# Illumina/strelka

Measured on AMD Instinct MI355X. Metric: candidate-alignment scoring cells/s (read bases x candidate alignments; Strelka2 has no pair-HMM, SURVEY.md section 0) + germline loci/s + 40x WGS-like germline wall-clock (e2e) + 110x/40x somatic wall-clock (e2e_somatic), higher is better.
Workload: dtype f64; 1 GPU; germline chr20-style synthetic (BASELINE.json configs[1]).  Headline: scoreCandidateAlignment as one function -- per GPU per step 65536 reads of 150 bp x 87.9 candidate alignments each (5-7 candidate indels around them), from the candidate alignments the device search left (PCal) to one double each: one kernel (F5: the walk of each alignment's path + the terms of its bases, penalties and clips).  ; read_len=150

## Files before the change

strelka_amd/csrc/read_enumerate.hip:

```cpp

#include "sk_common.h"

#include "align_entry.h"
#include "read_enumerate.h"

#include <algorithm>
#include <chrono>
#include <climits>
#include <cstdio>
#include <cstdlib>
#include <cstring>
#include <vector>

using namespace skcore;

int sk_score_alignments_launch_hostleg(const sk_align_batch* b, double* dev_out_lnp, void* hip_stream);

namespace
{

static_assert(sizeof(PFrame) % 4 == 0 && sizeof(PCal) % 4 == 0, "frames move through LDS as 32-bit words");


struct EnumArgs
// ... 337 lines not shown
            if (k <= a.light_cals) a.list[lat++] = r; else a.list[n - 1 - hat++] = r;
        }
        atomicMax(&a.dyn[DYN_MAX_CALS], max_cals);
        if (t == 0) {
            a.dyn[DYN_N_CALS] = total;
            a.dyn[DYN_N_LIGHT] = tot_light;
            a.dyn[DYN_N_HEAVY] = tot_heavy;
        }
    }
}


__device__ inline uint8_t code_of(const char c)
{
    switch (c) {
    case '=': return SK_BAM_REF;
    case 'A': return SK_BAM_A;
    case 'C': return SK_BAM_C;
    case 'G': return SK_BAM_G;
    case 'T': return SK_BAM_T;
    default: return SK_BAM_ANY;
    }
}

struct FlatArgs
{
    PJob job;
    const char* ins_pool;
    const char* ref;
    int32_t ref_offset, ref_len;
    int32_t n_reads, n_cals;
    const PCal* pool;
    const int32_t* list;
    int32_t* status;
    const int64_t* read_off;
    const uint8_t* read_code;
    const int32_t* cal_off;
    int32_t* win_begin;
    int32_t* win_end;
    int32_t* ins_lo;
    int32_t* ins_hi;
    uint8_t* n_seg8;
    int32_t* win_len;
    int32_t* hap_len;
    int32_t* n_ins;
    int16_t* ins_idx;
    int32_t* ins_off;
    int32_t* n_ops;
    const int64_t* hap_off;
    PCal* cals;
    uint8_t* hap_code;
    const int64_t* op_off;
// ... 291 lines not shown
            s_cal[k * REC_STRIDE + j] = v;
            dst[j] = v;
        }
    }
    __syncthreads();
    if (c >= a.n_cals) return;
    const int r = read_of_cal(a, c);
    const PCal& cal = *reinterpret_cast<const PCal*>(s_cal + lane * REC_STRIDE);
    if (a.status[r] != ST_OK) return;
    (void)flatten_cal<true>(a, r, cal, int32_t(a.read_off[r + 1] - a.read_off[r]), a.ops + a.op_off[c]);
    for (int i = 0; i < cal.n_indels; ++i) (void)job_cand(a.job, cal.indels[i]);
    if (cal.lead >= 0) (void)job_cand(a.job, cal.lead);
    if (cal.trail >= 0) (void)job_cand(a.job, cal.trail);
}

constexpr int F5_MAX_READ = 256;
constexpr int ONE_WAIT_MAX_READS = 16384;
constexpr int F5_MAX_POOL = 768;
#ifndef F5_SORT
#define F5_SORT 1
#endif
constexpr int F5_TAB = 32;

static_assert(F5_TAB <= 64, "the table copy is a lane an entry");

struct FusedScoreArgs
{
    FlatArgs f;
    const uint8_t* read_qual;
    const SkTables* tab;
    double* scores;
    unsigned* err;
    int32_t* n_unhandled;
    int32_t write_cals;
    unsigned long long* dbg;
    unsigned* queue;
};

constexpr int F5_SEGS = 16, F5_INDELS = 8;
constexpr int F5_SLOT = (F5_SEGS + 1) | 1;
__device__ __forceinline__ int f5_ent_word(const int k) { return k; }
constexpr int F5_ROW = 3;

struct F5Tab
{
    int32_t pos;
    uint32_t del, ins_len;
    uint32_t type_cand;
    int32_t ins_at;
};

template <int MAXR>
struct F5Lds
{
    uint8_t read[MAXR + 12];
    uint8_t hap[F5_MAX_POOL + 12];
    double row[(MAXR + 8) * F5_ROW];
    uint32_t slot[64 * F5_SLOT];
    F5Tab tab[F5_TAB];
};
static_assert(sizeof(F5Lds<152>) <= 10240, "sixteen waves of the short-read form to a CU");
static_assert(3 * 4 * sizeof(F5Lds<F5_MAX_READ>) <= 160 * 1024, "three four-wave blocks of the long-read form to a CU");
static_assert((152 + 12) % 4 == 0 && (F5_MAX_READ + 12) % 4 == 0 && (F5_MAX_POOL + 12) % 4 == 0, "the byte arrays' words stay aligned");
static_assert(INS_CAP <= 64, "a lane an insert");

struct F5Rec
{
    uint32_t w0, w1, w2;
    uint64_t types;
    uint64_t l0, l1, l2, l3;
    uint64_t ind;
    int ind_lo;
    __device__ __forceinline__ int32_t pos() const { return int32_t(w0); }
    __device__ __forceinline__ int lead() const { return int(int16_t(w1 & 0xffffu)); }
    __device__ __forceinline__ int trail() const { return int(int16_t(w1 >> 16)); }
    __device__ __forceinline__ int n_seg() const { return int((w2 >> 8) & 0xffu); }
    __device__ __forceinline__ int n_indels() const { return int((w2 >> 16) & 0xffu); }
    __device__ __forceinline__ int indel(const int k) const { return ind_lo + int(unsigned(ind >> (6 * k)) & 63u); }
};
static_assert(F5_TAB <= 64 && 6 * F5_INDELS <= 64, "an indel index in 6 bits, eight in one value");

template <typename LDS>
__device__ __forceinline__ int f5_walk_selects(LDS& S, const F5Rec c, const bool has, const int tab_lo, const int32_t win_begin, uint8_t* consulted,
                                               const int32_t L, const int32_t P, uint32_t* const myslot)
{
    constexpr uint64_t N1 = 0x1111111111111111ull;
    const uint64_t types = c.types, p_l0 = c.l0, p_l1 = c.l1, p_l2 = c.l2, p_l3 = c.l3;
    const int aps = has ? c.n_seg() : 0;
    auto eq4 = [=](const unsigned v) -> uint64_t {
        uint64_t x = types ^ (N1 * v);
        x |= x >> 1;
        x |= x >> 2;
        return ~x & N1;
    };
    auto seg_len = [=](const int i) -> unsigned {
        const uint64_t lo = (i & 4) ? p_l1 : p_l0, hi = (i & 4) ? p_l3 : p_l2;
        return unsigned(((i & 8) ? hi : lo) >> (16 * (i & 3))) & 0xffffu;
    };
    const uint64_t in_path = (aps >= 16) ? N1 : (((1ull << (4 * aps)) - 1ull) & N1);
    const uint64_t M4 = (eq4(SK_SEG_MATCH) | eq4(SK_SEG_SEQ_MATCH) | eq4(SK_SEG_SEQ_MISMATCH)) & in_path;
    const uint64_t I4 = eq4(SK_SEG_INSERT) & in_path, D4 = eq4(SK_SEG_DELETE) & in_path;
    const int ends_first = M4 ? (__builtin_ctzll(M4) >> 2) : aps, ends_second = M4 ? ((63 - __builtin_clzll(M4)) >> 2) : aps;
    const int ni = c.n_indels();
    int ni_wave = 0;
#pragma unroll
    for (int k = 1; k <= F5_INDELS; ++k) ni_wave = __any(ni >= k) ? k : ni_wave;
// ... 44 lines not shown
                else del_len += l;
            }
            read_step = ins_len;
            ref_step = del_len;
        }
        const unsigned asked = (del_len << 16) | ins_len;
        const bool askable = del_len < 0xffffu && ins_len < 0xffffu;
        int k_found = 0, n_found = 0;
        bool open = true;
#pragma unroll
        for (int k = 0; k < F5_INDELS; ++k) {
            if (k < ni_wave) {
                const bool m = open && k_pos[k] == ref_head_pos && k_pack[k] == asked;
                k_found = m ? k : k_found;
                n_found += m ? 1 : 0;
                open = open && (m || k_pos[k] <= ref_head_pos);
            }
        }
        int key = (n_found == 1) ? c.indel(k_found) : -2;
        key = (pi < ends_first) ? c.lead() : (pi > ends_second) ? c.trail() : key;
        const bool key_ok = key >= 0;
        const F5Tab te = S.tab[(key_ok ? key : tab_lo) - tab_lo];
        const bool indel_ok = live && is_indel_seg && key_ok;
        if (indel_ok && consulted) consulted[key] = 1;
        const bool pen = is_indel_seg && (te.type_cand >> 8) == 0u;
        const int32_t head = (pi < ends_first) ? int32_t(te.ins_len) - int32_t(ln) : 0;
        const bool ins_bases = is_indel_seg && ins_len > 0u;
        const bool ins_ok = ins_len <= 0xffffu && head >= 0 && uint32_t(head) + ins_len <= te.ins_len && te.ins_at >= 0;
        const bool bases = ins_bases || is_match;
        const int32_t src = ins_bases ? te.ins_at + head : ref_head_pos - win_begin;
        const unsigned len = ins_bases ? ins_len : ln;
        const bool known = is_indel_seg || is_match || is_clip || ty == SK_SEG_SKIP || ty == SK_SEG_HARD_CLIP;
        bool fail = !known || (is_indel_seg && (!key_ok || !askable)) || (ins_bases && !ins_ok);
        const bool entry = (bases || (is_clip && !is_indel_seg)) && len > 0u;
        if (entry) {
            fail = fail || pos + int32_t(len) > L || (bases && (src < 0 || int64_t(src) + int64_t(len) > int64_t(P)));
            const int hidx = bases ? int(src) - pos : 0;
            fail = fail || n_ent > F5_SEGS || npen > 4u || hidx < -256 || hidx > 3839;
            if (live && !fail) myslot[f5_ent_word(n_ent)] = unsigned(pos) | (npen << 9) | (bases ? 0u : 1u << 15) | (unsigned(hidx + 256) << 16);
        }
        if (live) {
            bad = fail;
            n_ent += entry ? 1 : 0;
            npen = entry ? (pen ? 1u : 0u) : npen + (pen ? 1u : 0u);
            pos += int32_t(read_step);
            ref_head_pos += int32_t(ref_step);
            pi += n_seg;
// ... 63 lines not shown
            const unsigned base = __umul24(unsigned(8 * F5_ROW), unsigned(p));
            double v[8];
#pragma unroll
            for (int u = 0; u < 8; ++u) {
                const unsigned at = base + unsigned(8 * F5_ROW * u) + ((sel[u >> 2] >> (8 * (u & 3))) & 0xffu);
                v[u] = *reinterpret_cast<const double*>(rows + at);
            }
#pragma unroll
            for (int u = 0; u < 8; ++u) lnp = __dadd_rn(lnp, v[u]);
            p += mm;
        }
        if (next_op()) break;
    }
    return lnp;
}

__device__ __forceinline__ void f5_wave_sync()
{
    __builtin_amdgcn_fence(__ATOMIC_RELEASE, "workgroup");
    __builtin_amdgcn_wave_barrier();
    __builtin_amdgcn_fence(__ATOMIC_ACQUIRE, "workgroup");
}

template <int MAXR, bool TIMING>
__device__ __forceinline__ void f5_read(const FusedScoreArgs& fa, const int r, F5Lds<MAXR>& S)
{
    auto now = [&]() -> unsigned long long { return TIMING ? (unsigned long long)clock64() : 0ull; };
    const FlatArgs& a = fa.f;
    const int lane = threadIdx.x & 63;
    const int c0 = a.cal_off[r], c1 = a.cal_off[r + 1];
    const int ncr = c1 - c0;
    if (ncr == 0 || a.status[r] != ST_OK) return;
    unsigned long long stamp[8];
    stamp[0] = now();
    const unsigned long long wall0 = TIMING ? (unsigned long long)wall_clock64() : 0ull;
    for (int i = 1; i < 8; ++i) stamp[i] = 0;
    const int64_t ro = a.read_off[r];
    const int32_t L = int32_t(a.read_off[r + 1] - ro);
    const int32_t P = a.hap_len[r];
    if (L > MAXR || P > F5_MAX_POOL) {
        if (lane == 0) atomicAdd(fa.n_unhandled, 1);
        return;
    }
    const int32_t win_begin = a.win_begin[r];
    const int n_ins = a.n_ins[r];
    int my_ins_idx = -1;
    int32_t my_ins_off = 0;
    {
        const int16_t* idx = a.ins_idx + size_t(r) * INS_CAP;
        const int32_t* off = a.ins_off + size_t(r) * INS_CAP;
        int32_t my_ins_len = 0;
        uint32_t my_ins_src = 0;
        if (lane < n_ins) {
            const int t_idx = idx[lane];
            my_ins_idx = t_idx;
            my_ins_off = off[lane];
            my_ins_len = int32_t(a.job.tab[t_idx].ins_len);
            my_ins_src = a.job.tab[t_idx].ins_off;
        }
        const int32_t win_len = a.win_len[r];
        for (int32_t i = lane; i < P + 8; i += 64) {
            uint8_t v = SK_BAM_ANY;
            if (i < win_len) {
                const int32_t p = win_begin + i;
                const bool outside = (p < a.ref_offset || p >= a.ref_offset + a.ref_len);
                if (outside && a.ref_outside) atomicAdd(a.ref_outside, 1);
                v = outside ? uint8_t(SK_BAM_ANY) : code_of(a.ref[p - a.ref_offset]);
            }
            S.hap[i] = v;
        }
        f5_wave_sync();
        for (int k = 0; k < n_ins; ++k) {
            const int32_t o = __builtin_amdgcn_readlane(my_ins_off, k), n = __builtin_amdgcn_readlane(my_ins_len, k);
            const uint32_t src = uint32_t(__builtin_amdgcn_readlane(int(my_ins_src), k));
            for (int32_t i = lane; i < n; i += 64)
                if (o + i < P) S.hap[o + i] = code_of(a.ins_pool[src + uint32_t(i)]);
        }
        const SkTables* __restrict__ T = fa.tab;
        for (int32_t i = lane; i < L + 12; i += 64) {
            unsigned q = 0;
            uint8_t code = SK_BAM_ANY;
            if (i < L) {
                code = a.read_code[ro + i];
                q = fa.read_qual[ro + i];
                if (q > 70u) {
                    atomicOr(fa.err, unsigned(SK_DEVERR_QSCORE));
                    q = 70u;
                }
            }
            S.read[i] = code & 15u;
            if (i < L + 8) {
                const unsigned c = code & 15u;
                const bool adds = i < L && c != 15u;
                const double agree = adds ? T->q2lncompe[q] : 0.0;
                S.row[F5_ROW * i] = agree;
                S.row[F5_ROW * i + 1] = 0.0;
                S.row[F5_ROW * i + 2] = !adds ? 0.0 : (c == 0u) ? agree : T->q2mis[q];
            }
        }
    }
    const double ln_quarter = fa.tab->ln_quarter, ln_noncand = fa.tab->ln_noncand;

    uint8_t* const order = S.hap + ((P + 8 + 3) & ~3);
    const bool sorted_order = (F5_SORT != 0) && ncr > 64 && ncr <= 256 && ((P + 8 + 3) & ~3) + ncr <= int(sizeof(S.hap));
    if (sorted_order) {
        int seg_of[4];
#pragma unroll
        for (int k = 0; k < 4; ++k) {
            const int j = lane + 64 * k;
            seg_of[k] = (j < ncr) ? int(a.n_seg8[c0 + j]) : -1;
            seg_of[k] = min(seg_of[k], F5_SEGS + 1);
        }
        unsigned present = 0;
#pragma unroll
        for (int k = 0; k < 4; ++k) present |= (seg_of[k] >= 0) ? (1u << seg_of[k]) : 0u;
#pragma unroll
        for (int d = 32; d >= 1; d >>= 1) present |= unsigned(__shfl_xor(int(present), d));
        present = unsigned(__builtin_amdgcn_readfirstlane(int(present)));
        int at = 0;
        while (present != 0u) {
            const int v = 31 - __builtin_clz(present);
            present &= ~(1u << v);
#pragma unroll
            for (int k = 0; k < 4; ++k) {
                const uint64_t m = __ballot(seg_of[k] == v);
                if (seg_of[k] == v) order[at + __popcll(m & ((1ull << lane) - 1ull))] = uint8_t(lane + 64 * k);
                at += __popcll(m);
            }
        }
    }

    for (int j0 = 0; j0 < ncr; j0 += 64) {
        const int nc = min(64, ncr - j0);
        f5_wave_sync();
        const unsigned long long ta = now();
        if (j0 == 0) stamp[1] = ta;
        const bool has = lane < nc;
        uint32_t* const myslot = S.slot + lane * F5_SLOT;
        bool fits = true;
        const int my_j = has ? (sorted_order ? int(order[j0 + lane]) : j0 + lane) : 0;
        F5Rec rec;
        rec.w0 = rec.w1 = rec.w2 = 0;
        rec.types = 0;
        rec.l0 = rec.l1 = rec.l2 = rec.l3 = 0;
        rec.ind = 0;
        rec.ind_lo = 0;
        uint64_t ind_raw0 = 0, ind_raw1 = 0;
        if (has) {
            const PCal* src = a.pool + a.list[c0 + my_j];
            const uint4* s4 = reinterpret_cast<const uint4*>(src);
            const uint4 q0 = s4[0], q1 = s4[1], q2 = s4[2], q3 = s4[3], q4 = s4[4];
            const uint32_t* si = reinterpret_cast<const uint32_t*>(src->indels);
            const uint32_t i0 = si[0], i1 = si[1], i2 = si[2], i3 = si[3];
            ind_raw0 = uint64_t(i0) | (uint64_t(i1) << 32);
            ind_raw1 = uint64_t(i2) | (uint64_t(i3) << 32);
            rec.w0 = q0.x;
            rec.w1 = q0.y;
            rec.w2 = q0.z;
            const unsigned nseg = (q0.z >> 8) & 0xffu, nind = (q0.z >> 16) & 0xffu;
            fits = (nseg <= unsigned(F5_SEGS) && nind <= unsigned(F5_INDELS));
            uint64_t types = 0;
            bool odd_type = false;
            auto pack4 = [&](const uint32_t a0, const uint32_t a1, const uint32_t a2, const uint32_t a3, const int first) -> uint64_t {
                types |= (uint64_t(a0 & 15u) | (uint64_t(a1 & 15u) << 4) | (uint64_t(a2 & 15u) << 8) | (uint64_t(a3 & 15u) << 12)) << (4 * first);
                odd_type = odd_type || (unsigned(first) < nseg && (a0 & 0xffffu) > 15u) || (unsigned(first + 1) < nseg && (a1 & 0xffffu) > 15u) ||
                           (unsigned(first + 2) < nseg && (a2 & 0xffffu) > 15u) || (unsigned(first + 3) < nseg && (a3 & 0xffffu) > 15u);
                return uint64_t(a0 >> 16) | (uint64_t(a1 >> 16) << 16) | (uint64_t(a2 >> 16) << 32) | (uint64_t(a3 >> 16) << 48);
            };
            rec.l0 = pack4(q0.w, q1.x, q1.y, q1.z, 0);
            rec.l1 = pack4(q1.w, q2.x, q2.y, q2.z, 4);
            rec.l2 = pack4(q2.w, q3.x, q3.y, q3.z, 8);
            rec.l3 = pack4(q3.w, q4.x, q4.y, q4.z, 12);
            rec.types = types;
            fits = fits && !odd_type;
        }
        auto raw_indel = [&](const int k) -> int { return int(int16_t(((k & 4) ? ind_raw1 : ind_raw0) >> (16 * (k & 3)))); };
        int tab_lo = 0;
        {
            int lo = INT_MAX, hi = INT_MIN;
            if (has && fits) {
                auto add = [&](const int i) {
                    lo = min(lo, i);
                    hi = max(hi, i);
                };
                const int ni = rec.n_indels();
                for (int i = 0; i < ni; ++i) add(raw_indel(i));
                if (rec.lead() >= 0) add(rec.lead());
                if (rec.trail() >= 0) add(rec.trail());
            }
#pragma unroll
            for (int d = 32; d > 0; d >>= 1) {
                lo = min(lo, __shfl_xor(lo, d));
                hi = max(hi, __shfl_xor(hi, d));
            }
            const int n_tab = (lo <= hi) ? hi - lo + 1 : 0;
            if (__any(has && !fits) || (n_tab > 0 && lo < 0) || n_tab > F5_TAB) {
                if (lane == 0) atomicAdd(fa.n_unhandled, 1);
                return;
            }
            tab_lo = n_tab ? lo : 0;
            uint64_t ind = 0;
#pragma unroll
            for (int k = 0; k < F5_INDELS; ++k) ind |= uint64_t(unsigned(raw_indel(k) - tab_lo) & 63u) << (6 * k);
            rec.ind = ind;
            rec.ind_lo = tab_lo;
            if (lane < n_tab) {
                const PIndel& g = a.job.tab[tab_lo + lane];
                F5Tab e;
                e.pos = g.pos;
                e.del = g.del;
                e.ins_len = g.ins_len;
                e.type_cand = unsigned(g.type) | (unsigned(g.cand) << 8);
                e.ins_at = -1;
                S.tab[lane] = e;
            }
            f5_wave_sync();
            if (my_ins_idx >= tab_lo && my_ins_idx < tab_lo + n_tab) S.tab[my_ins_idx - tab_lo].ins_at = my_ins_off;
        }
        f5_wave_sync();
        const unsigned long long tc = now();
        stamp[2] += tc - ta;
        int n_ent = 0;
        bool bad = false;
        {
            const unsigned long long tA0 = now();
            n_ent = f5_walk_selects(S, rec, has, tab_lo, win_begin, a.job.consulted, L, P, myslot);
            const unsigned long long tA1 = now();
            stamp[7] += tA1 - tA0;
            bad = n_ent < 0;
            if (has) {
                if (a.job.consulted) {
                    const int ni = rec.n_indels();
                    for (int i = 0; i < ni; ++i) a.job.consulted[rec.indel(i)] = 1;
                    if (rec.lead() >= 0) a.job.consulted[rec.lead()] = 1;
                    if (rec.trail() >= 0) a.job.consulted[rec.trail()] = 1;
                }
                if (bad) a.status[r] = ST_FAIL;
            }
            (void)tA1;
        }
        __builtin_amdgcn_wave_barrier();
        const unsigned long long td = now();
        stamp[4] += td - tc;
        if (has && !bad) {
            const double lnp = f5_sum(S, myslot, n_ent, ln_noncand, ln_quarter);
            fa.scores[c0 + my_j] = lnp;
        }
        stamp[5] += now() - td;
    }
    if (fa.dbg && lane == 0) {
        stamp[6] = now();
        stamp[3] = TIMING ? (unsigned long long)wall_clock64() - wall0 : 0ull;
        for (int i = 0; i < 8; ++i) fa.dbg[size_t(r) * 8 + i] = stamp[i];
    }
}

template <int MAXR, bool TIMING, int WAVES>
__global__ __launch_bounds__(64 * WAVES) __attribute__((amdgpu_waves_per_eu(4, 4))) void flatten_score_kernel(const FusedScoreArgs fa, const int n_reads)
{
    __shared__ __attribute__((aligned(16))) F5Lds<MAXR> S[WAVES];
    const int wave = threadIdx.x >> 6, lane = threadIdx.x & 63;
    for (;;) {
        int r = 0;
        if (lane == 0) r = int(atomicAdd(&fa.queue[0], 1u));
        r = __builtin_amdgcn_readfirstlane(r);
        if (r >= n_reads) break;
        f5_read<MAXR, TIMING>(fa, r, S[wave]);
        f5_wave_sync();
    }
    if (lane == 0) {
        __threadfence();
        if (atomicAdd(&fa.queue[1], 1u) == gridDim.x * unsigned(WAVES) - 1u) {
            fa.queue[0] = 0u;
            fa.queue[1] = 0u;
        }
    }
}

template <int MAXR, bool TIMING>
static void launch_flatten_score_t(const int n_reads, hipStream_t st, const FusedScoreArgs& fs)
{
    static const int waves = [] { const char* e = std::getenv("SK_F5_WAVES"); return e ? std::atoi(e) : 0; }();
    constexpr int DEFAULT_WAVES = (sizeof(F5Lds<MAXR>) * 16 <= 160 * 1024) ? 8 : 4;
    const int w = waves > 0 ? waves : DEFAULT_WAVES;
    static const int grid_env = [] { const char* e = std::getenv("SK_F5_GRID"); return e ? std::atoi(e) : 0; }();
    constexpr int WAVES_PER_CU = int((160 * 1024) / sizeof(F5Lds<MAXR>)) >= 16 ? 16 : int((160 * 1024) / sizeof(F5Lds<MAXR>));
    auto grid = [&](const int wpb) {
        const int resident = grid_env > 0 ? grid_env : 256 * std::max(1, WAVES_PER_CU / wpb);
        return dim3(unsigned(std::max(1, std::min(resident, (n_reads + wpb - 1) / wpb))));
    };
// ... 481 lines not shown
    {
        if (bytes <= cap) return 0;
        if (p) (void)skrt::hostFree(p);
        p = nullptr;
        cap = 0;
        const size_t want = bytes + bytes / 4 + 4096;
        SK_HIP(skrt::hostMalloc(&p, want));
        cap = want;
        return 0;
    }
    template <typename T> T* as() const { return static_cast<T*>(p); }
};

struct View
{
    void* p = nullptr;
    template <typename T> T* as() const { return static_cast<T*>(p); }
};

struct EnumBuffers
{
    DevBuf in_arena, zero_arena, minmax_arena, mask_arena;
    HostBuf h_in_arena, h_zero_arena;
    View tab, ins, toggle, ref, reads, read_off, read_code, read_qual, r2i, i2r, orig, map_level;
    View counters, status, warn, n_raw, hap_len, fill, n_uniq, consulted;
    View win_begin, ins_lo, win_end, ins_hi, evmask, addmask;
    View h_counters, h_status, h_warn, h_n_raw, h_hap_len, h_n_uniq, h_consulted;
    View cal_off_z, h_cal_off_z;
    DevBuf level_a, level_b, pool, leaf_read, leaf_hash;
    DevBuf raw_off, grouped, ghash, gkey, dup, sorted;
    DevBuf n_ops, win_len, n_ins, ins_idx, ins_off, n_seg8;
    DevBuf cal_off, hap_off, cals, hap_code, op_off, ops, entries, scores, colmat, colmat_off;
    DevBuf s3_order, s3_smooth, s3_flag, s3_rm_type, s3_rm_pos, s3_key, s3_sorted_score, s3_sorted_hash, s3_next_same, s3_range_end, s3_removed, s3_out, s3_list;
    HostBuf h_s3_out, h_s3_list;
    HostBuf h_raw_off, h_n_ops, h_cal_off, h_hap_off, h_op_off, h_cals, h_scores, h_colmat_off;
};
EnumBuffers& bufs()
{
    static EnumBuffers b;
    return b;
}

}

extern "C" int sk_enum_device_available(void) { return sk_ctx().ready ? 1 : 0; }

namespace
// ... 136 lines not shown
        size_t bytes, off;
    };
    auto lay_out = [](Piece* pc, const int n_pieces) {
        size_t at = 0;
        for (int i = 0; i < n_pieces; ++i) {
            pc[i].off = at;
            at += (pc[i].bytes + 255) & ~size_t(255);
        }
        return at;
    };
    Piece ins_p[] = {
        { &B.tab, in->tab, sizeof(PIndel) * size_t(in->n_tab), 0 },
        { &B.ins, in->ins_pool, size_t(in->ins_pool_len), 0 },
        { &B.toggle, in->max_toggle, sizeof(uint32_t) * size_t(in->n_max_toggle), 0 },
        { &B.ref, in->ref, size_t(std::max(in->ref_len, 0)), 0 },
        { &B.reads, in->reads, sizeof(PRead) * size_t(n), 0 },
        { &B.read_off, in->read_off, sizeof(int64_t) * size_t(n + 1), 0 },
        { &B.read_code, in->read_code, size_t(n_bases), 0 },
        { &B.read_qual, in->read_qual, size_t(n_bases), 0 },
        { &B.r2i, in->r2i, with_stage3 ? 8 * size_t(in->n_tab) : 0, 0 },
        { &B.i2r, in->i2r, with_stage3 ? 8 * size_t(in->n_tab) : 0, 0 },
        { &B.orig, in->orig, with_stage3 ? 4 * size_t(in->n_tab) : 0, 0 },
        { &B.map_level, in->map_level, with_stage3 ? 4 * size_t(n) : 0, 0 },
    };
    const int n_ins_p = int(sizeof(ins_p) / sizeof(ins_p[0]));
    const size_t in_bytes = lay_out(ins_p, n_ins_p);
    Piece zero_p[] = {
        { &B.counters, nullptr, 4 * size_t(n_counters), 0 }, { &B.warn, nullptr, 4 * size_t(n), 0 },    { &B.n_raw, nullptr, 4 * size_t(n), 0 },
        { &B.status, nullptr, 4 * size_t(n), 0 },            { &B.hap_len, nullptr, 4 * size_t(n), 0 }, { &B.fill, nullptr, 4 * size_t(n), 0 },
        { &B.n_uniq, nullptr, 4 * size_t(n), 0 },            { &B.consulted, nullptr, size_t(in->n_tab) + 1, 0 },
        { &B.cal_off_z, nullptr, one_wait ? 4 * size_t(n + 1) : 0, 0 },
    };
    View* zero_host[] = { &B.h_counters, &B.h_warn, &B.h_n_raw, &B.h_status, &B.h_hap_len, nullptr, &B.h_n_uniq, &B.h_consulted, &B.h_cal_off_z };
    const int n_zero_p = int(sizeof(zero_p) / sizeof(zero_p[0]));
    const size_t zero_bytes = lay_out(zero_p, n_zero_p);
    Piece minmax_p[] = { { &B.win_begin, nullptr, 4 * size_t(n), 0 }, { &B.ins_lo, nullptr, 4 * size_t(n), 0 },
                         { &B.win_end, nullptr, 4 * size_t(n), 0 },   { &B.ins_hi, nullptr, 4 * size_t(n), 0 } };
    const size_t minmax_bytes = lay_out(minmax_p, 4);
    Piece mask_p[] = { { &B.evmask, nullptr, 4 * (size_t(n) * size_t(W) + 1), 0 }, { &B.addmask, nullptr, 4 * (size_t(n) * size_t(W) + 1), 0 } };
    const size_t mask_bytes = lay_out(mask_p, 2);
    RES(in_arena, in_bytes);
    RES(zero_arena, zero_bytes);
    RES(minmax_arena, minmax_bytes);
    RES(mask_arena, mask_bytes);
    HRES(h_in_arena, in_bytes);
    HRES(h_zero_arena, zero_bytes);
    for (int i = 0; i < n_ins_p; ++i) {
        ins_p[i].view->p = static_cast<char*>(B.in_arena.p) + ins_p[i].off;
        if (ins_p[i].bytes) std::memcpy(static_cast<char*>(B.h_in_arena.p) + ins_p[i].off, ins_p[i].src, ins_p[i].bytes);
    }
    for (int i = 0; i < n_zero_p; ++i) {
        zero_p[i].view->p = static_cast<char*>(B.zero_arena.p) + zero_p[i].off;
        if (zero_host[i]) zero_host[i]->p = static_cast<char*>(B.h_zero_arena.p) + zero_p[i].off;
    }
    for (int i = 0; i < 4; ++i) minmax_p[i].view->p = static_cast<char*>(B.minmax_arena.p) + minmax_p[i].off;
    for (int i = 0; i < 2; ++i) mask_p[i].view->p = static_cast<char*>(B.mask_arena.p) + mask_p[i].off;
    auto fetch_zero = [&](const View& first, const View& last, const size_t last_bytes) -> int {
        const size_t a0 = size_t(static_cast<char*>(first.p) - static_cast<char*>(B.zero_arena.p));
        const size_t a1 = size_t(static_cast<char*>(last.p) - static_cast<char*>(B.zero_arena.p)) + last_bytes;
        SK_HIP(skrt::memcpyAsync(static_cast<char*>(B.h_zero_arena.p) + a0, static_cast<char*>(B.zero_arena.p) + a0, a1 - a0, hipMemcpyDeviceToHost, st));
        return 0;
    };

#define H2D(buf, src, bytes) \
    if ((bytes) > 0) SK_HIP(skrt::memcpyAsync(B.buf.p, src, size_t(bytes), hipMemcpyHostToDevice, st))
#define D2H(hbuf, buf, bytes) \
    if ((bytes) > 0) SK_HIP(skrt::memcpyAsync(B.hbuf.p, B.buf.p, size_t(bytes), hipMemcpyDeviceToHost, st))
    static const bool stage_by_kernel = !(std::getenv("SK_ENUM_STAGE_COPIES") != nullptr);
    if (one_wait && stage_by_kernel) {
        const uint32_t n_in16 = uint32_t(in_bytes / 16), n_zero16 = uint32_t(zero_bytes / 16);
        const int blocks = int(std::min<size_t>(std::max<size_t>((std::max(in_bytes, zero_bytes) / 16 + 255) / 256, 1), 256));
        SK_LAUNCH(job_stage_in_kernel, dim3(blocks), dim3(256), 0, st, static_cast<const uint4*>(B.h_in_arena.p), static_cast<uint4*>(B.in_arena.p), n_in16,
// ... 128 lines not shown
        sa.sorted = B.sorted.as<int32_t>();
        const int e2_blocks = int(std::min<int64_t>(std::max<int64_t>((int64_t(n) * 64 + 255) / 256, 8), 2048));
        SK_LAUNCH(group_kernel, dim3(e2_blocks), dim3(256), 0, st, sa);
        SK_LAUNCH(dedupe_kernel, dim3(e2_blocks), dim3(256), 0, st, sa);
        int light_cals = S3_LIGHT_CALS, lds_cals = S3_LDS_CALS;
        if (const char* e = std::getenv("SK_STAGE3_TEST_LDS_CALS")) {
            int a = 0, b = 0;
            if (std::sscanf(e, "%d,%d", &a, &b) == 2 && a > 0 && b >= a && b <= S3_LDS_CALS) {
                light_cals = a;
                lds_cals = b;
            }
        }
        sc.count = B.n_uniq.as<int32_t>();
        sc.off = B.cal_off_z.as<int32_t>();
        sc.list = B.s3_list.as<int32_t>();
        sc.light_cals = light_cals;
        SK_LAUNCH(job_scan_kernel<true>, dim3(1), dim3(1024), 0, st, sc);
        SK_LAUNCH(rank_kernel, dim3(e2_blocks), dim3(256), 0, st, sa);
        FlatArgs fa;
        std::memset(&fa, 0, sizeof(fa));
        fa.job = dj;
        fa.ins_pool = B.ins.as<char>();
        fa.ref = B.ref.as<char>();
        fa.ref_offset = in->ref_offset;
        fa.ref_len = in->ref_len;
        fa.n_reads = n;
        fa.n_cals = n_cap;
        fa.n_cals_on_device = 1;
        fa.pool = ea.pool;
        fa.list = B.sorted.as<int32_t>();
        fa.status = ea.status;
        fa.read_off = B.read_off.as<int64_t>();
        fa.read_code = B.read_code.as<uint8_t>();
        fa.cal_off = B.cal_off_z.as<int32_t>();
        fa.win_begin = B.win_begin.as<int32_t>();
        fa.win_len = B.win_len.as<int32_t>();
        fa.hap_len = B.hap_len.as<int32_t>();
        fa.n_ins = B.n_ins.as<int32_t>();
        fa.ins_idx = B.ins_idx.as<int16_t>();
        fa.ins_off = B.ins_off.as<int32_t>();
        fa.win_end = B.win_end.as<int32_t>();
        fa.ins_lo = B.ins_lo.as<int32_t>();
        fa.ins_hi = B.ins_hi.as<int32_t>();
        fa.n_seg8 = B.n_seg8.as<uint8_t>();
        fa.max_read_len = in->max_read_len;
        fa.ref_outside = dyn + DYN_REF_OUTSIDE;
// ... 191 lines not shown
        SK_HIP(skrt::getLastError());
    }
    if (fetch_zero(B.n_uniq, B.n_uniq, 4 * size_t(n))) return 1;
    SK_HIP(skrt::streamSynchronize(st));
    const int32_t* h_n_uniq = B.h_n_uniq.as<int32_t>();
    for (int r = 0; r < n; ++r) h_cal_off[r + 1] = h_cal_off[r] + ((h_status[r] == ST_OK) ? h_n_uniq[r] : 0);
    const int32_t n_cals = h_cal_off[n];
    SK_HIP(skrt::memcpyAsync(B.cal_off.p, h_cal_off, 4 * size_t(n + 1), hipMemcpyHostToDevice, st));
    if (n_grouped > 0) {
        SK_LAUNCH(rank_kernel, dim3((n_grouped + 255) / 256), dim3(256), 0, st, sa);
        SK_HIP(skrt::getLastError());
    }
    lap("E2 sets");

    RES(n_ops, 4 * size_t(n_cals));
    RES(op_off, 8 * size_t(n_cals + 1));
    HRES(h_n_ops, 4 * size_t(n_cals));
    HRES(h_op_off, 8 * size_t(n_cals + 1));
    FlatArgs fa;
    std::memset(&fa, 0, sizeof(fa));
    fa.job = dj;
    fa.ins_pool = B.ins.as<char>();
    fa.ref = B.ref.as<char>();
    fa.ref_offset = in->ref_offset;
    fa.ref_len = in->ref_len;
    fa.n_reads = n;
    fa.n_cals = n_cals;
    fa.pool = ea.pool;
    fa.list = B.sorted.as<int32_t>();
    fa.status = ea.status;
    fa.read_off = B.read_off.as<int64_t>();
    fa.read_code = B.read_code.as<uint8_t>();
    fa.cal_off = B.cal_off.as<int32_t>();
    fa.win_begin = B.win_begin.as<int32_t>();
    fa.win_len = B.win_len.as<int32_t>();
    fa.hap_len = B.hap_len.as<int32_t>();
    fa.n_ins = B.n_ins.as<int32_t>();
    fa.ins_idx = B.ins_idx.as<int16_t>();
    fa.ins_off = B.ins_off.as<int32_t>();
    fa.n_ops = B.n_ops.as<int32_t>();
    fa.win_end = B.win_end.as<int32_t>();
    fa.ins_lo = B.ins_lo.as<int32_t>();
    fa.ins_hi = B.ins_hi.as<int32_t>();
    RES(n_seg8, size_t(n_cals));
    fa.n_seg8 = B.n_seg8.as<uint8_t>();
    fa.ref_outside = B.counters.as<int32_t>() + (Caps::K + 8 + DYN_REF_OUTSIDE);
// ... 373 lines not shown
```

Baseline: 762.0 billion cells/s.

## Precode reference and inserts on host, batch per-read loads, bitmask consulted flags

Reference and insert-pool bases are converted to BAM codes once on the host into padded device arrays, so the kernel reads four codes per word instead of branching per byte. Per-read metadata, read codes and qualities, candidate list entries and the whole indel table are loaded into registers up front, and the next candidate record is prefetched, so global latencies overlap instead of serializing. Quality terms are cached in LDS per block, and consulted-indel writes become a wave-reduced bitmask with one check-then-write per entry. The cost is more registers per lane, extra host preprocessing and device memory, and a separate path for tables larger than 32 entries.

New measurement: 817.5 billion cells/s (median of 6 runs). 7.3% higher.

```diff
diff --git a/strelka_amd/csrc/read_enumerate.hip b/strelka_amd/csrc/read_enumerate.hip
--- a/strelka_amd/csrc/read_enumerate.hip
+++ b/strelka_amd/csrc/read_enumerate.hip
@@ -383,12 +383,33 @@
     default: return SK_BAM_ANY;
     }
 }
+constexpr int F5_CODE_PAD = 1024;
+struct CodeLut
+{
+    uint8_t code[256];
+    CodeLut()
+    {
+        std::memset(code, SK_BAM_ANY, sizeof(code));
+        code[uint8_t('=')] = SK_BAM_REF;
+        code[uint8_t('A')] = SK_BAM_A;
+        code[uint8_t('C')] = SK_BAM_C;
+        code[uint8_t('G')] = SK_BAM_G;
+        code[uint8_t('T')] = SK_BAM_T;
+    }
+};
+inline const CodeLut& code_lut()
+{
+    static const CodeLut l;
+    return l;
+}
 
 struct FlatArgs
 {
     PJob job;
     const char* ins_pool;
     const char* ref;
+    const uint8_t* ref_code;
+    const uint8_t* ins_code;
     int32_t ref_offset, ref_len;
     int32_t n_reads, n_cals;
     const PCal* pool;
@@ -726,7 +747,7 @@
 #endif
 constexpr int F5_TAB = 32;
 
-static_assert(F5_TAB <= 64, "the table copy is a lane an entry");
+static_assert(F5_TAB <= 32, "the table copy is a lane an entry, the consulted mask a bit an entry");
 
 struct FusedScoreArgs
 {
@@ -763,10 +784,16 @@
     uint32_t slot[64 * F5_SLOT];
     F5Tab tab[F5_TAB];
 };
-static_assert(sizeof(F5Lds<152>) <= 10240, "sixteen waves of the short-read form to a CU");
-static_assert(3 * 4 * sizeof(F5Lds<F5_MAX_READ>) <= 160 * 1024, "three four-wave blocks of the long-read form to a CU");
+constexpr int F5_Q_TERMS = 2 * (SK_NQ + 1);
+constexpr size_t f5_block_granules(const size_t lds_object, const int waves)
+{
+    return (lds_object * size_t(waves) + 8 * size_t(F5_Q_TERMS) + 1279) / 1280;
+}
+static_assert(sizeof(F5Lds<152>) <= 10240 && 2 * f5_block_granules(sizeof(F5Lds<152>), 8) <= 128, "two eight-wave blocks of the short-read form to a CU");
+static_assert(3 * f5_block_granules(sizeof(F5Lds<F5_MAX_READ>), 4) <= 128, "three four-wave blocks of the long-read form to a CU");
 static_assert((152 + 12) % 4 == 0 && (F5_MAX_READ + 12) % 4 == 0 && (F5_MAX_POOL + 12) % 4 == 0, "the byte arrays' words stay aligned");
 static_assert(INS_CAP <= 64, "a lane an insert");
+static_assert(F5_CODE_PAD >= F5_MAX_POOL + 16 && F5_CODE_PAD % 4 == 0, "a window that leaves the reference stays inside the pad");
 
 struct F5Rec
 {
@@ -782,10 +809,10 @@
     __device__ __forceinline__ int n_indels() const { return int((w2 >> 16) & 0xffu); }
     __device__ __forceinline__ int indel(const int k) const { return ind_lo + int(unsigned(ind >> (6 * k)) & 63u); }
 };
-static_assert(F5_TAB <= 64 && 6 * F5_INDELS <= 64, "an indel index in 6 bits, eight in one value");
+static_assert(6 * F5_INDELS <= 64, "an indel index in 6 bits, eight in one value");
 
 template <typename LDS>
-__device__ __forceinline__ int f5_walk_selects(LDS& S, const F5Rec c, const bool has, const int tab_lo, const int32_t win_begin, uint8_t* consulted,
+__device__ __forceinline__ int f5_walk_selects(LDS& S, const F5Rec c, const bool has, const int tab_lo, const int32_t win_begin, uint32_t& consulted,
                                                const int32_t L, const int32_t P, uint32_t* const myslot)
 {
     constexpr uint64_t N1 = 0x1111111111111111ull;
@@ -876,7 +903,7 @@
         const bool key_ok = key >= 0;
         const F5Tab te = S.tab[(key_ok ? key : tab_lo) - tab_lo];
         const bool indel_ok = live && is_indel_seg && key_ok;
-        if (indel_ok && consulted) consulted[key] = 1;
+        consulted |= indel_ok ? (1u << ((key - tab_lo) & 31)) : 0u;
         const bool pen = is_indel_seg && (te.type_cand >> 8) == 0u;
         const int32_t head = (pi < ends_first) ? int32_t(te.ins_len) - int32_t(ln) : 0;
         const bool ins_bases = is_indel_seg && ins_len > 0u;
@@ -986,95 +1013,131 @@
     __builtin_amdgcn_fence(__ATOMIC_ACQUIRE, "workgroup");
 }
 
+struct F5Raw
+{
+    uint4 q0, q1, q2, q3, q4;
+    uint32_t i0, i1, i2, i3;
+};
+__device__ __forceinline__ F5Raw f5_load_raw(const PCal* src)
+{
+    F5Raw w;
+    const uint4* s4 = reinterpret_cast<const uint4*>(src);
+    w.q0 = s4[0], w.q1 = s4[1], w.q2 = s4[2], w.q3 = s4[3], w.q4 = s4[4];
+    const uint32_t* si = reinterpret_cast<const uint32_t*>(src->indels);
+    w.i0 = si[0], w.i1 = si[1], w.i2 = si[2], w.i3 = si[3];
+    return w;
+}
+
+constexpr int F5_INS_REG = 4;
+
 template <int MAXR, bool TIMING>
-__device__ __forceinline__ void f5_read(const FusedScoreArgs& fa, const int r, F5Lds<MAXR>& S)
+__device__ __forceinline__ void f5_read(const FusedScoreArgs& fa, const int r, F5Lds<MAXR>& S, const double* const q_terms)
 {
     auto now = [&]() -> unsigned long long { return TIMING ? (unsigned long long)clock64() : 0ull; };
     const FlatArgs& a = fa.f;
-    const int lane = threadIdx.x & 63;
-    const int c0 = a.cal_off[r], c1 = a.cal_off[r + 1];
-    const int ncr = c1 - c0;
-    if (ncr == 0 || a.status[r] != ST_OK) return;
+    int lane_of_read = threadIdx.x & 63;
+    __asm__ volatile("" : "+v"(lane_of_read));
+    const int lane = lane_of_read;
     unsigned long long stamp[8];
     stamp[0] = now();
     const unsigned long long wall0 = TIMING ? (unsigned long long)wall_clock64() : 0ull;
+    int g1_c0 = a.cal_off[r], g1_c1 = a.cal_off[r + 1];
+    int32_t g1_status = a.status[r];
+    int64_t g1_ro = a.read_off[r], g1_ro1 = a.read_off[r + 1];
+    int32_t g1_P = a.hap_len[r], g1_win_begin = a.win_begin[r], g1_n_ins = a.n_ins[r], g1_win_len = a.win_len[r];
+    __asm__ volatile("" : "+v"(g1_c0), "+v"(g1_c1), "+v"(g1_status), "+v"(g1_ro), "+v"(g1_ro1), "+v"(g1_P), "+v"(g1_win_begin), "+v"(g1_n_ins), "+v"(g1_win_len));
+    auto uniform64 = [](const int64_t v) -> int64_t {
+        return int64_t(uint64_t(uint32_t(__builtin_amdgcn_readfirstlane(int(uint32_t(uint64_t(v)))))) |
+                       (uint64_t(uint32_t(__builtin_amdgcn_readfirstlane(int(uint32_t(uint64_t(v) >> 32))))) << 32));
+    };
+    const int c0 = __builtin_amdgcn_readfirstlane(g1_c0), c1 = __builtin_amdgcn_readfirstlane(g1_c1);
+    const int32_t status_r = __builtin_amdgcn_readfirstlane(g1_status);
+    const int64_t ro = uniform64(g1_ro), ro1 = uniform64(g1_ro1);
+    const int32_t P = __builtin_amdgcn_readfirstlane(g1_P);
+    const int32_t win_begin = __builtin_amdgcn_readfirstlane(g1_win_begin);
+    const int n_ins = __builtin_amdgcn_readfirstlane(g1_n_ins);
+    const int32_t win_len = __builtin_amdgcn_readfirstlane(g1_win_len);
+    const double ln_quarter = fa.tab->ln_quarter, ln_noncand = fa.tab->ln_noncand;
+    const int ncr = c1 - c0;
+    if (ncr == 0 || status_r != ST_OK) return;
     for (int i = 1; i < 8; ++i) stamp[i] = 0;
-    const int64_t ro = a.read_off[r];
-    const int32_t L = int32_t(a.read_off[r + 1] - ro);
-    const int32_t P = a.hap_len[r];
+    const int32_t L = int32_t(ro1 - ro);
     if (L > MAXR || P > F5_MAX_POOL) {
         if (lane == 0) atomicAdd(fa.n_unhandled, 1);
         return;
     }
-    const int32_t win_begin = a.win_begin[r];
-    const int n_ins = a.n_ins[r];
+    const int job_n_tab = a.job.n_tab;
+    const bool whole_tab = job_n_tab <= F5_TAB;
+    uint8_t* const order = S.hap + ((P + 8 + 3) & ~3);
+    const bool sorted_order = (F5_SORT != 0) && ncr > 64 && ncr <= 256 && ((P + 8 + 3) & ~3) + ncr <= int(sizeof(S.hap));
+    int32_t slot_next = 0;
+    if (!sorted_order && lane < ncr) slot_next = a.list[c0 + lane];
+    int32_t lst[4];
+#pragma unroll
+    for (int k = 0; k < 4; ++k) {
+        lst[k] = 0;
+        if (sorted_order && lane + 64 * k < ncr) lst[k] = a.list[c0 + lane + 64 * k];
+    }
+    F5Tab g;
+    g.pos = 0, g.del = 0, g.ins_len = 0, g.type_cand = 0, g.ins_at = -1;
+    uint32_t g_ins_off = 0;
+    if (whole_tab && lane < job_n_tab) {
+        const PIndel& e = a.job.tab[lane];
+        g.pos = e.pos;
+        g.del = e.del;
+        g.ins_len = e.ins_len;
+        g.type_cand = unsigned(e.type) | (unsigned(e.cand) << 8);
+        g_ins_off = e.ins_off;
+    }
     int my_ins_idx = -1;
     int32_t my_ins_off = 0;
+    if (lane < n_ins) {
+        my_ins_idx = a.ins_idx[size_t(r) * INS_CAP + lane];
+        my_ins_off = a.ins_off[size_t(r) * INS_CAP + lane];
+    }
+    constexpr int HAP_WORDS = int(sizeof(S.hap)) / 4, HAP_K = (HAP_WORDS + 63) / 64;
+    constexpr uint32_t ANY4 = 0x01010101u * uint32_t(SK_BAM_ANY);
+    uint32_t hw[HAP_K];
     {
-        const int16_t* idx = a.ins_idx + size_t(r) * INS_CAP;
-        const int32_t* off = a.ins_off + size_t(r) * INS_CAP;
-        int32_t my_ins_len = 0;
-        uint32_t my_ins_src = 0;
-        if (lane < n_ins) {
-            const int t_idx = idx[lane];
-            my_ins_idx = t_idx;
-            my_ins_off = off[lane];
-            my_ins_len = int32_t(a.job.tab[t_idx].ins_len);
-            my_ins_src = a.job.tab[t_idx].ins_off;
-        }
-        const int32_t win_len = a.win_len[r];
-        for (int32_t i = lane; i < P + 8; i += 64) {
-            uint8_t v = SK_BAM_ANY;
-            if (i < win_len) {
-                const int32_t p = win_begin + i;
-                const bool outside = (p < a.ref_offset || p >= a.ref_offset + a.ref_len);
-                if (outside && a.ref_outside) atomicAdd(a.ref_outside, 1);
-                v = outside ? uint8_t(SK_BAM_ANY) : code_of(a.ref[p - a.ref_offset]);
-            }
-            S.hap[i] = v;
-        }
-        f5_wave_sync();
-        for (int k = 0; k < n_ins; ++k) {
-            const int32_t o = __builtin_amdgcn_readlane(my_ins_off, k), n = __builtin_amdgcn_readlane(my_ins_len, k);
-            const uint32_t src = uint32_t(__builtin_amdgcn_readlane(int(my_ins_src), k));
-            for (int32_t i = lane; i < n; i += 64)
-                if (o + i < P) S.hap[o + i] = code_of(a.ins_pool[src + uint32_t(i)]);
-        }
-        const SkTables* __restrict__ T = fa.tab;
-        for (int32_t i = lane; i < L + 12; i += 64) {
-            unsigned q = 0;
-            uint8_t code = SK_BAM_ANY;
-            if (i < L) {
-                code = a.read_code[ro + i];
-                q = fa.read_qual[ro + i];
-                if (q > 70u) {
-                    atomicOr(fa.err, unsigned(SK_DEVERR_QSCORE));
-                    q = 70u;
-                }
-            }
-            S.read[i] = code & 15u;
-            if (i < L + 8) {
-                const unsigned c = code & 15u;
-                const bool adds = i < L && c != 15u;
-                const double agree = adds ? T->q2lncompe[q] : 0.0;
-                S.row[F5_ROW * i] = agree;
-                S.row[F5_ROW * i + 1] = 0.0;
-                S.row[F5_ROW * i + 2] = !adds ? 0.0 : (c == 0u) ? agree : T->q2mis[q];
-            }
-        }
-    }
-    const double ln_quarter = fa.tab->ln_quarter, ln_noncand = fa.tab->ln_noncand;
-
-    uint8_t* const order = S.hap + ((P + 8 + 3) & ~3);
-    const bool sorted_order = (F5_SORT != 0) && ncr > 64 && ncr <= 256 && ((P + 8 + 3) & ~3) + ncr <= int(sizeof(S.hap));
+        const int32_t p_max = int32_t(min(int64_t(a.ref_len) + F5_CODE_PAD - 4, int64_t(INT_MAX - 2 * F5_CODE_PAD)));
+        const int32_t wbase = int32_t(min(max(int64_t(win_begin) - int64_t(a.ref_offset), int64_t(-2 * F5_CODE_PAD)), int64_t(p_max) + F5_CODE_PAD));
+#pragma unroll
+        for (int k = 0; k < HAP_K; ++k) {
+            const int w = lane + 64 * k;
+            hw[k] = ANY4;
+            if (4 * w < win_len) {
+                const int32_t p = min(max(wbase + 4 * w, -F5_CODE_PAD), p_max);
+                uint32_t v;
+                __builtin_memcpy(&v, a.ref_code + p, 4);
+                hw[k] = v;
+            }
+        }
+    }
+    constexpr int READ_K = (MAXR + 12 + 63) / 64;
+    uint8_t rc[READ_K], rq[READ_K];
+#pragma unroll
+    for (int k = 0; k < READ_K; ++k) {
+        const int i = lane + 64 * k;
+        rc[k] = SK_BAM_ANY;
+        rq[k] = 0;
+        if (i < L) {
+            rc[k] = a.read_code[ro + i];
+            rq[k] = fa.read_qual[ro + i];
+        }
+    }
+    uint8_t seg8[4];
+#pragma unroll
+    for (int k = 0; k < 4; ++k) {
+        seg8[k] = 0;
+        if (sorted_order && lane + 64 * k < ncr) seg8[k] = a.n_seg8[c0 + lane + 64 * k];
+    }
     if (sorted_order) {
+#pragma unroll
+        for (int k = 0; k < 4; ++k)
+            if (lane + 64 * k < ncr) S.slot[lane + 64 * k] = uint32_t(lst[k]);
         int seg_of[4];
 #pragma unroll
-        for (int k = 0; k < 4; ++k) {
-            const int j = lane + 64 * k;
-            seg_of[k] = (j < ncr) ? int(a.n_seg8[c0 + j]) : -1;
-            seg_of[k] = min(seg_of[k], F5_SEGS + 1);
-        }
+        for (int k = 0; k < 4; ++k) seg_of[k] = (lane + 64 * k < ncr) ? min(int(seg8[k]), F5_SEGS + 1) : -1;
         unsigned present = 0;
 #pragma unroll
         for (int k = 0; k < 4; ++k) present |= (seg_of[k] >= 0) ? (1u << seg_of[k]) : 0u;
@@ -1090,6 +1153,96 @@
                 const uint64_t m = __ballot(seg_of[k] == v);
                 if (seg_of[k] == v) order[at + __popcll(m & ((1ull << lane) - 1ull))] = uint8_t(lane + 64 * k);
                 at += __popcll(m);
+            }
+        }
+        f5_wave_sync();
+        slot_next = int32_t(S.slot[order[lane]]);
+    }
+    int32_t my_ins_len = 0;
+    uint32_t my_ins_src = 0;
+    if (whole_tab) {
+        const int32_t len_t = __shfl(int32_t(g.ins_len), my_ins_idx & 63);
+        const uint32_t src_t = uint32_t(__shfl(int(g_ins_off), my_ins_idx & 63));
+        if (lane < n_ins) {
+            my_ins_len = len_t;
+            my_ins_src = src_t;
+        }
+    } else if (lane < n_ins) {
+        my_ins_len = int32_t(a.job.tab[my_ins_idx].ins_len);
+        my_ins_src = a.job.tab[my_ins_idx].ins_off;
+    }
+    const bool ins_in_regs = n_ins <= F5_INS_REG && !__any(my_ins_len > 64);
+    uint32_t ib[F5_INS_REG];
+    int32_t ib_n[F5_INS_REG];
+    uint32_t ib_src[F5_INS_REG];
+#pragma unroll
+    for (int k = 0; k < F5_INS_REG; ++k) {
+        ib_n[k] = ins_in_regs ? __builtin_amdgcn_readlane(my_ins_len, k) : 0;
+        ib_src[k] = uint32_t(__builtin_amdgcn_readlane(int(my_ins_src), k));
+    }
+#pragma unroll
+    for (int k = 0; k < F5_INS_REG; ++k) {
+        ib[k] = SK_BAM_ANY;
+        if (lane < ib_n[k]) ib[k] = a.ins_code[ib_src[k] + uint32_t(lane)];
+    }
+    F5Raw raw0 = f5_load_raw(a.pool + slot_next);
+    if (a.ref_outside && lane == 0) {
+        const int64_t b = max(int64_t(win_begin), int64_t(a.ref_offset));
+        const int64_t e = min(int64_t(win_begin) + int64_t(win_len), int64_t(a.ref_offset) + int64_t(a.ref_len));
+        const int32_t outside = win_len - int32_t(max(e - b, int64_t(0)));
+        if (outside > 0) atomicAdd(a.ref_outside, outside);
+    }
+    {
+        uint32_t* const hap_w = reinterpret_cast<uint32_t*>(S.hap);
+        const int n_words = (P + 8 + 3) >> 2;
+#pragma unroll
+        for (int k = 0; k < HAP_K; ++k) {
+            const int w = lane + 64 * k;
+            const int keep = win_len - 4 * w;
+            const uint32_t m = (keep >= 4) ? 0xffffffffu : (keep <= 0) ? 0u : ((1u << (8 * keep)) - 1u);
+            if (w < n_words) hap_w[w] = (hw[k] & m) | (ANY4 & ~m);
+        }
+    }
+    if (whole_tab) {
+        if (lane < job_n_tab) S.tab[lane] = g;
+        f5_wave_sync();
+        if (lane < n_ins && my_ins_idx < job_n_tab) S.tab[my_ins_idx].ins_at = my_ins_off;
+    }
+    f5_wave_sync();
+    if (ins_in_regs) {
+#pragma unroll
+        for (int k = 0; k < F5_INS_REG; ++k) {
+            if (k < n_ins) {
+                const int32_t o = __builtin_amdgcn_readlane(my_ins_off, k), n = __builtin_amdgcn_readlane(my_ins_len, k);
+                if (lane < n && o + lane < P) S.hap[o + lane] = uint8_t(ib[k]);
+            }
+        }
+    } else {
+        for (int k = 0; k < n_ins; ++k) {
+            const int32_t o = __builtin_amdgcn_readlane(my_ins_off, k), n = __builtin_amdgcn_readlane(my_ins_len, k);
+            const uint32_t src = uint32_t(__builtin_amdgcn_readlane(int(my_ins_src), k));
+            for (int32_t i = lane; i < n; i += 64)
+                if (o + i < P) S.hap[o + i] = a.ins_code[src + uint32_t(i)];
+        }
+    }
+#pragma unroll
+    for (int k = 0; k < READ_K; ++k) {
+        const int32_t i = lane + 64 * k;
+        if (i < L + 12) {
+            unsigned q = rq[k];
+            const uint8_t code = rc[k];
+            if (q > 70u) {
+                atomicOr(fa.err, unsigned(SK_DEVERR_QSCORE));
+                q = 70u;
+            }
+            S.read[i] = code & 15u;
+            if (i < L + 8) {
+                const unsigned c = code & 15u;
+                const bool adds = i < L && c != 15u;
+                const double agree = adds ? q_terms[q] : 0.0;
+                S.row[F5_ROW * i] = agree;
+                S.row[F5_ROW * i + 1] = 0.0;
+                S.row[F5_ROW * i + 2] = !adds ? 0.0 : (c == 0u) ? agree : q_terms[SK_NQ + 1 + q];
             }
         }
     }
@@ -1110,14 +1263,12 @@
         rec.ind = 0;
         rec.ind_lo = 0;
         uint64_t ind_raw0 = 0, ind_raw1 = 0;
+        if (j0 > 0) raw0 = f5_load_raw(a.pool + slot_next);
         if (has) {
-            const PCal* src = a.pool + a.list[c0 + my_j];
-            const uint4* s4 = reinterpret_cast<const uint4*>(src);
-            const uint4 q0 = s4[0], q1 = s4[1], q2 = s4[2], q3 = s4[3], q4 = s4[4];
-            const uint32_t* si = reinterpret_cast<const uint32_t*>(src->indels);
-            const uint32_t i0 = si[0], i1 = si[1], i2 = si[2], i3 = si[3];
-            ind_raw0 = uint64_t(i0) | (uint64_t(i1) << 32);
-            ind_raw1 = uint64_t(i2) | (uint64_t(i3) << 32);
+            const F5Raw w = raw0;
+            const uint4 q0 = w.q0, q1 = w.q1, q2 = w.q2, q3 = w.q3, q4 = w.q4;
+            ind_raw0 = uint64_t(w.i0) | (uint64_t(w.i1) << 32);
+            ind_raw1 = uint64_t(w.i2) | (uint64_t(w.i3) << 32);
             rec.w0 = q0.x;
             rec.w1 = q0.y;
             rec.w2 = q0.z;
@@ -1140,7 +1291,25 @@
         }
         auto raw_indel = [&](const int k) -> int { return int(int16_t(((k & 4) ? ind_raw1 : ind_raw0) >> (16 * (k & 3)))); };
         int tab_lo = 0;
-        {
+        if (whole_tab) {
+            bool out_of_table = false;
+            if (has && fits) {
+                auto check = [&](const int i) { out_of_table = out_of_table || i < 0 || i >= job_n_tab; };
+                const int ni = rec.n_indels();
+                for (int i = 0; i < ni; ++i) check(raw_indel(i));
+                if (rec.lead() >= 0) check(rec.lead());
+                if (rec.trail() >= 0) check(rec.trail());
+            }
+            if (__any((has && !fits) || out_of_table)) {
+                if (lane == 0) atomicAdd(fa.n_unhandled, 1);
+                return;
+            }
+            uint64_t ind = 0;
+#pragma unroll
+            for (int k = 0; k < F5_INDELS; ++k) ind |= uint64_t(unsigned(raw_indel(k)) & 63u) << (6 * k);
+            rec.ind = ind;
+            rec.ind_lo = 0;
+        } else {
             int lo = INT_MAX, hi = INT_MIN;
             if (has && fits) {
                 auto add = [&](const int i) {
@@ -1186,23 +1355,31 @@
         stamp[2] += tc - ta;
         int n_ent = 0;
         bool bad = false;
+        bool cons_mine = false;
+        uint8_t cons_seen = 1;
         {
             const unsigned long long tA0 = now();
-            n_ent = f5_walk_selects(S, rec, has, tab_lo, win_begin, a.job.consulted, L, P, myslot);
+            uint32_t cons = 0;
+            n_ent = f5_walk_selects(S, rec, has, tab_lo, win_begin, cons, L, P, myslot);
             const unsigned long long tA1 = now();
             stamp[7] += tA1 - tA0;
             bad = n_ent < 0;
             if (has) {
-                if (a.job.consulted) {
-                    const int ni = rec.n_indels();
-                    for (int i = 0; i < ni; ++i) a.job.consulted[rec.indel(i)] = 1;
-                    if (rec.lead() >= 0) a.job.consulted[rec.lead()] = 1;
-                    if (rec.trail() >= 0) a.job.consulted[rec.trail()] = 1;
-                }
+                const int ni = rec.n_indels();
+                for (int i = 0; i < ni; ++i) cons |= 1u << ((rec.indel(i) - tab_lo) & 31);
+                if (rec.lead() >= 0) cons |= 1u << ((rec.lead() - tab_lo) & 31);
+                if (rec.trail() >= 0) cons |= 1u << ((rec.trail() - tab_lo) & 31);
                 if (bad) a.status[r] = ST_FAIL;
             }
+            if (a.job.consulted) {
+#pragma unroll
+                for (int d = 32; d > 0; d >>= 1) cons |= uint32_t(__shfl_xor(int(cons), d));
+                cons_mine = lane < 32 && ((cons >> lane) & 1u) != 0u;
+                if (cons_mine) cons_seen = a.job.consulted[tab_lo + lane];
+            }
             (void)tA1;
         }
+        if (j0 + 64 + lane < ncr) slot_next = a.list[c0 + (sorted_order ? int(order[j0 + 64 + lane]) : j0 + 64 + lane)];
         __builtin_amdgcn_wave_barrier();
         const unsigned long long td = now();
         stamp[4] += td - tc;
@@ -1210,6 +1387,9 @@
             const double lnp = f5_sum(S, myslot, n_ent, ln_noncand, ln_quarter);
             fa.scores[c0 + my_j] = lnp;
         }
+        if (cons_mine && cons_seen == 0) a.job.consulted[tab_lo + lane] = 1;
+        raw0.q0 = raw0.q1 = raw0.q2 = raw0.q3 = raw0.q4 = make_uint4(0, 0, 0, 0);
+        raw0.i0 = raw0.i1 = raw0.i2 = raw0.i3 = 0;
         stamp[5] += now() - td;
     }
     if (fa.dbg && lane == 0) {
@@ -1223,13 +1403,16 @@
 __global__ __launch_bounds__(64 * WAVES) __attribute__((amdgpu_waves_per_eu(4, 4))) void flatten_score_kernel(const FusedScoreArgs fa, const int n_reads)
 {
     __shared__ __attribute__((aligned(16))) F5Lds<MAXR> S[WAVES];
+    __shared__ double q_terms[F5_Q_TERMS];
+    for (int i = threadIdx.x; i < F5_Q_TERMS; i += 64 * WAVES) q_terms[i] = (i <= SK_NQ) ? fa.tab->q2lncompe[i] : fa.tab->q2mis[i - (SK_NQ + 1)];
+    __syncthreads();
     const int wave = threadIdx.x >> 6, lane = threadIdx.x & 63;
     for (;;) {
         int r = 0;
         if (lane == 0) r = int(atomicAdd(&fa.queue[0], 1u));
         r = __builtin_amdgcn_readfirstlane(r);
         if (r >= n_reads) break;
-        f5_read<MAXR, TIMING>(fa, r, S[wave]);
+        f5_read<MAXR, TIMING>(fa, r, S[wave], q_terms);
         f5_wave_sync();
     }
     if (lane == 0) {
@@ -1757,7 +1940,7 @@
 {
     DevBuf in_arena, zero_arena, minmax_arena, mask_arena;
     HostBuf h_in_arena, h_zero_arena;
-    View tab, ins, toggle, ref, reads, read_off, read_code, read_qual, r2i, i2r, orig, map_level;
+    View tab, ins, toggle, ref, ref_code, ins_code, reads, read_off, read_code, read_qual, r2i, i2r, orig, map_level;
     View counters, status, warn, n_raw, hap_len, fill, n_uniq, consulted;
     View win_begin, ins_lo, win_end, ins_hi, evmask, addmask;
     View h_counters, h_status, h_warn, h_n_raw, h_hap_len, h_n_uniq, h_consulted;
@@ -1940,6 +2123,8 @@
         { &B.i2r, in->i2r, with_stage3 ? 8 * size_t(in->n_tab) : 0, 0 },
         { &B.orig, in->orig, with_stage3 ? 4 * size_t(in->n_tab) : 0, 0 },
         { &B.map_level, in->map_level, with_stage3 ? 4 * size_t(n) : 0, 0 },
+        { &B.ref_code, nullptr, size_t(std::max(in->ref_len, 0)) + 2 * size_t(F5_CODE_PAD), 0 },
+        { &B.ins_code, nullptr, size_t(in->ins_pool_len), 0 },
     };
     const int n_ins_p = int(sizeof(ins_p) / sizeof(ins_p[0]));
     const size_t in_bytes = lay_out(ins_p, n_ins_p);
@@ -1965,7 +2150,17 @@
     HRES(h_zero_arena, zero_bytes);
     for (int i = 0; i < n_ins_p; ++i) {
         ins_p[i].view->p = static_cast<char*>(B.in_arena.p) + ins_p[i].off;
-        if (ins_p[i].bytes) std::memcpy(static_cast<char*>(B.h_in_arena.p) + ins_p[i].off, ins_p[i].src, ins_p[i].bytes);
+        if (ins_p[i].bytes && ins_p[i].src) std::memcpy(static_cast<char*>(B.h_in_arena.p) + ins_p[i].off, ins_p[i].src, ins_p[i].bytes);
+    }
+    {
+        const CodeLut& lut = code_lut();
+        const size_t ref_n = size_t(std::max(in->ref_len, 0));
+        uint8_t* rc = static_cast<uint8_t*>(B.h_in_arena.p) + size_t(static_cast<char*>(B.ref_code.p) - static_cast<char*>(B.in_arena.p));
+        std::memset(rc, SK_BAM_ANY, size_t(F5_CODE_PAD));
+        for (size_t i = 0; i < ref_n; ++i) rc[size_t(F5_CODE_PAD) + i] = lut.code[uint8_t(in->ref[i])];
+        std::memset(rc + size_t(F5_CODE_PAD) + ref_n, SK_BAM_ANY, size_t(F5_CODE_PAD));
+        uint8_t* ic = static_cast<uint8_t*>(B.h_in_arena.p) + size_t(static_cast<char*>(B.ins_code.p) - static_cast<char*>(B.in_arena.p));
+        for (size_t i = 0; i < size_t(in->ins_pool_len); ++i) ic[i] = lut.code[uint8_t(in->ins_pool[i])];
     }
     for (int i = 0; i < n_zero_p; ++i) {
         zero_p[i].view->p = static_cast<char*>(B.zero_arena.p) + zero_p[i].off;
@@ -2140,6 +2335,8 @@
         fa.job = dj;
         fa.ins_pool = B.ins.as<char>();
         fa.ref = B.ref.as<char>();
+        fa.ref_code = B.ref_code.as<uint8_t>() + F5_CODE_PAD;
+        fa.ins_code = B.ins_code.as<uint8_t>();
         fa.ref_offset = in->ref_offset;
         fa.ref_len = in->ref_len;
         fa.n_reads = n;
@@ -2377,6 +2574,8 @@
     fa.job = dj;
     fa.ins_pool = B.ins.as<char>();
     fa.ref = B.ref.as<char>();
+    fa.ref_code = B.ref_code.as<uint8_t>() + F5_CODE_PAD;
+    fa.ins_code = B.ins_code.as<uint8_t>();
     fa.ref_offset = in->ref_offset;
     fa.ref_len = in->ref_len;
     fa.n_reads = n;
```
